# e4s2022/e4s

Hardware: AMD Instinct MI355X
Metric: 1024^2 face-swap images/sec (higher is better)
Workload: dtype f32 operands as hi+lo bf16, 3 bf16 MFMAs per product, f32 accumulate (bf16x3) on the 3x3 convs whose launch fills the chip; exact f32 elsewhere; 1 GPU; E4S-core face swap at 1024^2 (2x Net3 encoder @256^2, style swap, 12 LocalMLPs, mask-guided StyleGAN2 generator K=13), BASELINE.json configs[3] shard: 8 swaps per GPU per step; per_gpu_batch=8, global_batch=8, out_size=1024, hip_graph=True, precision=as bf16x3 where the launch fills the chip (this batch), else exact fp32, parallelism=image-parallel x1

## Files before the change

e4s_amd/csrc/conv_bf16x3.hip:

```cpp
#include "common.h"
#include <stdlib.h>

namespace {

typedef __bf16 bf16x8 __attribute__((ext_vector_type(8)));
typedef float f32x8 __attribute__((ext_vector_type(8)));

constexpr int KC = 32;
constexpr int ROWB = 144;
constexpr int LO = 64;
constexpr int TW = 16, HALO_W = TW + 2;
constexpr int PBM = 256, PTH = 16, PHALO = (PTH + 2) * HALO_W;
constexpr int PNTHR = 512;

template <int BN_, int WM_, int WN_, int TPS_, int KCH_ = 32>
struct PCfg {
    static constexpr int BN = BN_, WM = WM_, WN = WN_, TPS = TPS_, KCH = KCH_;
    static constexpr int TM = PBM / (WM * 32), TN = BN / (WN * 32);
    static constexpr int ROWB = KCH == 32 ? 144 : 80;
    static constexpr int LO = KCH * 2;
    static constexpr int QG = KCH / 8;
    static constexpr int KSTEPS = KCH / 16;
    static constexpr int ITEMS = PHALO * QG;
    static constexpr int A_BYTES = PHALO * ROWB;
// ... 43 lines not shown
    if (want > nchunk / 2) want = nchunk / 2;
    if (want < 2) return;
    cper = (nchunk + want - 1) / want;
    ksplit = (nchunk + cper - 1) / cper;
}

inline void region_split(const e4s_conv_params& p, int& ksplit, int& cper) {
    const int64_t tiles = (int64_t)p.B * ((p.Ha + 15) / 16) * ((p.Wa + 15) / 16) * p.ncls * (p.Cout / 128);
    few_tiles_split(tiles, p.Cin / 32, ksplit, cper);
}

struct TileId {
    int tb, tyb, txb, n0, ks, c_lo, c_hi;
};

template <typename C, int XF, bool SHUF, int VAR = 0>
__global__ __launch_bounds__(PNTHR) void conv_bf16x3_kernel(const e4s_conv_params p, const int ntn, const int tx_n,
                                                            const int per_img, const int ntiles, const int ksplit,
                                                            const int cper) {
    constexpr int BM = PBM, BN = C::BN, NTHR = PNTHR, WN = C::WN, TM = C::TM, TN = C::TN, TH = PTH, TPS = C::TPS;
    constexpr int NSTG = C::NSTG, PIECE = C::PIECE, BITEMS = C::BITEMS, BJ = C::BJ;
    constexpr int A_BYTES = C::A_BYTES, B_BYTES = C::B_BYTES, NZ = SHUF ? 4 : 1;
    constexpr int KC = C::KCH, ROWB = C::ROWB, LO = C::LO, QG = C::QG, KSTEPS = C::KSTEPS, BPC = C::BPC, PITEMS = C::ITEMS;
    extern __shared__ __attribute__((aligned(16))) unsigned char smem[];
    unsigned char* sA = smem;
    unsigned char* sB = smem + 2 * A_BYTES;
    int* s_out = reinterpret_cast<int*>(sB + 2 * B_BYTES);
    float* s_nz = reinterpret_cast<float*>(s_out + 3 * BM);
    double* s_st = reinterpret_cast<double*>(s_nz + 3 * BM * NZ);

    const int tid = threadIdx.x;
    const int lane = tid & 63, wave = tid >> 6;
    const int li = lane & 31, kh = lane >> 5;
    const int wm = wave / WN, wn = wave % WN;
// ... 271 lines not shown
                osc[tn] = p.out_scale ? p.out_scale[(size_t)cur.tb * p.Cout + co] : 1.f;
                bsv[tn] = p.bias ? p.bias[co] : 0.f;
                slp[tn] = (p.act == 2) ? p.slope[co] : p.alpha;
                coff[tn] = ((ph >> 1) * p.Wo + (ph & 1)) * ycs + co;
                nzi[tn] = ph;
            }
            const float gain = (p.act == 1) ? p.gain : 1.f;
            const bool do_act = p.act != 0;
            const bool raw = ksplit > 1;
            const bool stats = !SHUF && !raw && p.stats_ws != nullptr;
            double st_s[TN], st_q[TN];
#pragma unroll
            for (int tn = 0; tn < TN; ++tn) st_s[tn] = st_q[tn] = 0.0;
            float* yo = raw ? p.splitk_ws + (size_t)cur.ks * ((size_t)p.B * p.Ho * p.Wo * ycs) : p.y;
            const bool wide = (ycs & 3) == 0;
#pragma unroll
            for (int tm = 0; tm < TM; ++tm) {
#pragma unroll
                for (int g = 0; g < 4; ++g) {
                    float v[TN][4];
#pragma unroll
                    for (int i = 0; i < 4; ++i) {
                        const int r = 4 * g + i;
                        const int row = (wm * TM + tm) * 32 + i + 8 * g + 4 * kh;
                        const bool live = so[row] >= 0;
#pragma unroll
                        for (int tn = 0; tn < TN; ++tn) {
                            float t = acc[tm][tn][r];
                            if (!raw) {
                                t = t * osc[tn] + sn[row * NZ + (SHUF ? nzi[tn] : 0)] + bsv[tn];
// ... 1 lines not shown
                            }
                            v[tn][i] = t;
                            if (stats && live) { st_s[tn] += (double)t; st_q[tn] += (double)t * (double)t; }
                        }
                    }
                    if (wide) {
#pragma unroll
                        for (int tn = 0; tn < TN; ++tn) quad_transpose4(v[tn][0], v[tn][1], v[tn][2], v[tn][3], li);
                        const int off = so[(wm * TM + tm) * 32 + (li & 3) + 8 * g + 4 * kh];
                        if (off >= 0) {
#pragma unroll
                            for (int tn = 0; tn < TN; ++tn)
                                *reinterpret_cast<f32x4*>(yo + (size_t)off * ycs + coff[tn] - (li & 3)) =
                                    f32x4{v[tn][0], v[tn][1], v[tn][2], v[tn][3]};
                        }
                    } else {
#pragma unroll
                        for (int i = 0; i < 4; ++i) {
                            const int off = so[(wm * TM + tm) * 32 + i + 8 * g + 4 * kh];
                            if (off < 0) continue;
#pragma unroll
                            for (int tn = 0; tn < TN; ++tn) yo[(size_t)off * ycs + coff[tn]] = v[tn][i];
                        }
                    }
                }
            }
            if (!SHUF && stats) {
#pragma unroll
                for (int tn = 0; tn < TN; ++tn) {
                    st_s[tn] += __shfl_xor(st_s[tn], 32, 64);
                    st_q[tn] += __shfl_xor(st_q[tn], 32, 64);
                    if (kh == 0) {
                        const int col = (wn * TN + tn) * 32 + li;
                        s_st[(wm * BN + col) * 2] = st_s[tn];
                        s_st[(wm * BN + col) * 2 + 1] = st_q[tn];
                    }
                }
// ... 680 lines not shown
    few_tiles_split(tiles, p.Cin / KC, ksplit, cper);
}

int num_cus() {
    static int cus[64] = {0};
    int dev = 0;
    if (hipGetDevice(&dev) != hipSuccess) return 256;
    if (!cus[dev & 63]) {
        hipDeviceProp_t prop;
        cus[dev & 63] = (hipGetDeviceProperties(&prop, dev) == hipSuccess && prop.multiProcessorCount > 0)
                            ? prop.multiProcessorCount : 256;
    }
    return cus[dev & 63];
}

template <typename C, int XF, bool SHUF, int VAR = 0>
int launch(const e4s_conv_params& p, hipStream_t st) {
    auto kern = conv_bf16x3_kernel<C, XF, SHUF, VAR>;
    constexpr int SMEM = plain_smem<C, SHUF>();
    static_assert(SMEM <= 160 * 1024, "LDS budget");
    static std::atomic<uint64_t> smem_set{0};
    if (int e = e4s_ensure_dyn_smem(reinterpret_cast<const void*>(kern), SMEM, smem_set)) return e;
    const int ngemm = SHUF ? 4 * p.Cout : p.Cout;
    const int ntn = ngemm / C::BN;
    const int tx_n = (p.Wa + TW - 1) / TW, per_img = ((p.Ha + PTH - 1) / PTH) * tx_n;
    int ksplit, cper;
    plain_split(p, ngemm / C::BN, ksplit, cper);
    cper *= 32 / C::KCH;
    if (ksplit > 1 && !p.splitk_ws) return (int)hipErrorInvalidValue;
    const int64_t ntiles = (int64_t)p.B * per_img * ntn * ksplit;
    if (ntiles <= 0) return 0;
    if (ntiles >= (1ll << 31)) return (int)hipErrorInvalidValue;
    const int grid = (int)(ntiles < num_cus() ? ntiles : num_cus());
    hipLaunchKernelGGL(kern, dim3((unsigned)grid), dim3(PNTHR), SMEM, st, p, ntn, tx_n, per_img, (int)ntiles, ksplit, cper);
    E4S_CHECK_LAUNCH();
    if (ksplit > 1) {
        const int ycs = p.y_cstride ? p.y_cstride : p.Cout;
        const int64_t npix = (int64_t)p.B * p.Ho * p.Wo;
        const int64_t n4 = npix * (p.Cout / 4);
        hipLaunchKernelGGL(splitk_epilogue_kernel, dim3((unsigned)((n4 + 255) / 256)), dim3(256), 0, st, p, ksplit, ycs,
                           (int64_t)p.Ho * p.Wo, n4);
        E4S_CHECK_LAUNCH();
    }
    return 0;
}

template <typename C, bool SHUF>
int launch_xf(const e4s_conv_params& p, hipStream_t st) {
    if (p.in_stats) return SHUF ? (int)hipErrorInvalidValue : launch<C, 2, false>(p, st);
// ... 46 lines not shown
    }
#endif
    if (up) {
        if ((4 * p.Cout) % 128) return (int)hipErrorInvalidValue;
        return launch_xf<CfgL, true>(p, st);
    }
#ifdef E4S_ABLATIONS
    static const int k16 = [] { const char* e = getenv("E4S_PLAIN_K16"); return e ? atoi(e) : 1; }();
    if (p.Cout % 128 == 0 && !k16) return launch_xf<CfgL, false>(p, st);
#endif
    if (p.Cout % 128 == 0) return launch_xf<CfgL16, false>(p, st);
    if (p.Cout % 64 == 0) return launch_xf<CfgM, false>(p, st);
    return launch_xf<CfgS, false>(p, st);
}

int e4s_splitk_epilogue(const e4s_conv_params& p, int ksplit, hipStream_t st) {
    if (!p.splitk_ws || ksplit < 2 || p.Cout % 4) return (int)hipErrorInvalidValue;
    e4s_conv_params q = p;
    q.out_scale = nullptr;
    const int ycs = p.y_cstride ? p.y_cstride : p.Cout;
    const int64_t n4 = (int64_t)p.B * p.Ho * p.Wo * (p.Cout / 4);
    hipLaunchKernelGGL(splitk_epilogue_kernel, dim3((unsigned)((n4 + 255) / 256)), dim3(256), 0, st, q, ksplit, ycs,
                       (int64_t)p.Ho * p.Wo, n4);
    E4S_CHECK_LAUNCH();
    return 0;
}

extern "C" int64_t e4s_conv_bf16x3_ws_floats(const e4s_conv_params* pp) {
    const e4s_conv_params& p = *pp;
    if (p.istride != 1 || p.ntaps != 9 || p.Cin % KC) return 0;
// ... 24 lines not shown
```

e4s_amd/csrc/conv_c32.hip:

```cpp
#include "common.h"
#include <stdlib.h>

namespace {

typedef __bf16 bf16x8 __attribute__((ext_vector_type(8)));
typedef float f32x8 __attribute__((ext_vector_type(8)));

constexpr int KC = 32, ROWB = 128, LO = 64;
constexpr int TW = 16, TH = 16, HALO_W = TW + 2, HALO = (TH + 2) * HALO_W;
constexpr int BM = TH * TW, BN = 32, NTHR = 256;
constexpr int ITEMS = HALO * 4, AJ = (ITEMS + NTHR - 1) / NTHR;
constexpr int BPIECES = 9 * BN * 8, BJ = BPIECES / NTHR;
constexpr int A_BYTES = HALO * ROWB, B_BYTES = 9 * BN * ROWB;
constexpr int YLD = 36;
constexpr int SMEM = B_BYTES + A_BYTES + BM * 8 + 3 * BN * 4;
static_assert(BPIECES % NTHR == 0 && BM == NTHR, "thread layout");
static_assert(BM * YLD * 4 <= A_BYTES, "the output staging tile aliases the halo buffer");
static_assert(2 * SMEM <= 160 * 1024, "two blocks per CU");

__device__ __forceinline__ int swz(int r, int g) { return r * ROWB + ((g ^ ((r >> 1) & 7)) << 4); }
__device__ __forceinline__ int swz_halo(int h, int g) { return h * ROWB + ((g ^ (((h % HALO_W) >> 1) & 7)) << 4); }

__device__ __forceinline__ void split_store(unsigned char* base, int off, const f32x8 v) {
    const bf16x8 h = __builtin_convertvector(v, bf16x8);
// ... 163 lines not shown
        const float osc = p.out_scale ? p.out_scale[(size_t)cur.tb * p.Cout + co] : 1.f;
        const float bsv = p.bias ? p.bias[co] : 0.f;
        const float gain = (p.act == 1) ? p.gain : 1.f;
        const int ycs = p.y_cstride ? p.y_cstride : p.Cout;
        __syncthreads();
#pragma unroll
        for (int tm = 0; tm < 2; ++tm)
#pragma unroll
            for (int r = 0; r < 16; ++r) {
                const int row = wave * 64 + tm * 32 + (r & 3) + 8 * (r >> 2) + 4 * kh;
                float v = acc[tm][r] * osc + s_nz[row] + bsv;
                if (p.act) v = (v > 0.f ? v : v * p.alpha) * gain;
                sY[row * YLD + li] = v;
            }
        __syncthreads();
        {
            const int c4 = tid & 7;
#pragma unroll
            for (int ps = 0; ps < BM / (NTHR / 8); ++ps) {
                const int px = ps * (NTHR / 8) + (tid >> 3);
                const int off = s_out[px];
                if (off >= 0 && abl != 3)
                    *reinterpret_cast<f32x4*>(p.y + (size_t)off * ycs + cur.nt * BN + c4 * 4) =
                        *reinterpret_cast<const f32x4*>(sY + px * YLD + c4 * 4);
            }
        }
        if (RGB) {
#pragma unroll
            for (int pass = 0; pass < 2; ++pass) {
                const int px = pass * (NTHR / 2) + (tid >> 1), hf = tid & 1;
                const float* yp = sY + px * YLD + hf * 16;
// ... 126 lines not shown
    hipLaunchKernelGGL(kern, dim3((unsigned)grid), dim3(NTHR), SMEM, st, p, rgb_ws, rgb_partial, ntn, tx_n, per_img, (int)ntiles,
                       abl);
    E4S_CHECK_LAUNCH();
    return 0;
}

}

extern "C" int e4s_conv_c32_bf16x3_f32(const e4s_conv_params* pp, const float* rgb_ws, float* rgb_partial, void* stream) {
    const e4s_conv_params& p = *pp;
    if (p.Cin != KC || p.Cout % BN || p.ntaps != 9 || p.ncls != 1 || p.istride != 1 || p.ostride != 1 || p.tiles || p.labels ||
        p.in_stats || p.noise_per_channel || p.act == 2 || p.Ho != p.Hi || p.Wo != p.Wi || p.B <= 0 || p.stats_ws)
        return (int)hipErrorInvalidValue;
    if ((rgb_ws == nullptr) != (rgb_partial == nullptr) || (rgb_ws && p.Cout != BN)) return (int)hipErrorInvalidValue;
    if ((int64_t)p.B * p.Ho * p.Wo >= (1ll << 31)) return (int)hipErrorInvalidValue;
    hipStream_t st = as_stream(stream);
    if (p.in_scale) return rgb_ws ? launch<1, 1>(p, rgb_ws, rgb_partial, st) : launch<1, 0>(p, rgb_ws, rgb_partial, st);
    return rgb_ws ? launch<0, 1>(p, rgb_ws, rgb_partial, st) : launch<0, 0>(p, rgb_ws, rgb_partial, st);
}

extern "C" int e4s_torgb_finish_f32(const float* partial, const float* bias, const float* skip, const float* k4, float* out, int B,
                                    int H, int W, void* stream) {
    if (!partial || !bias || !out || (skip && (!k4 || ((H | W) & 1)))) return (int)hipErrorInvalidValue;
    if (B <= 0 || H <= 0 || W <= 0) return 0;
    const int W4 = (W + 3) / 4, HP = (H + 1) / 2;
    const int64_t n = (int64_t)B * 3 * HP * W4;
    if ((n + 255) / 256 >= (1ll << 31)) return (int)hipErrorInvalidValue;
    hipLaunchKernelGGL(torgb_finish_kernel, dim3((unsigned)((n + 255) / 256)), dim3(256), 0, as_stream(stream), partial, bias, skip, k4,
                       out, H, W, W4, HP, n);
    E4S_CHECK_LAUNCH();
    return 0;
// ... 2 lines not shown
```

e4s_amd/csrc/ops.hip:

```cpp
#include "common.h"

namespace {

__device__ __forceinline__ float bias_act_one(float x, float ref, int code, float alpha, float scale) {
    float y;
    switch (code) {
        case 12: case 32: y = 0.f; break;
        case 30: y = (x > 0.f) ? x : x * alpha; break;
        case 31: y = (ref > 0.f) ? x : x * alpha; break;
        default: y = x; break;
    }
    return y * scale;
}

__global__ void fused_bias_act_v4(const f32x4* __restrict__ x, const float* __restrict__ b,
                                  const f32x4* __restrict__ ref, f32x4* __restrict__ y, int64_t n4,
                                  int step_b, int size_b, int code, float alpha, float scale) {
    const int64_t stride = (int64_t)gridDim.x * blockDim.x;
    for (int64_t i = (int64_t)blockIdx.x * blockDim.x + threadIdx.x; i < n4; i += stride) {
        f32x4 v = x[i];
        if (b) {
            const float bv = b[((i * 4) / step_b) % size_b];
            v += bv;
        }
// ... 75 lines not shown
        if (oy >= out_h || ox >= out_w) continue;
        const int my = oy * down_y - pad_y0, mx = ox * down_x - pad_x0;
        const int iy_first = floordiv(my + up_y - 1, up_y), ix_first = floordiv(mx + up_x - 1, up_x);
        float acc = 0.f;
        for (int iy = iy_first, jy = iy_first * up_y - my; jy < kh; ++iy, jy += up_y) {
            const float* row = sx + (iy - in_y0) * tin_w;
            for (int ix = ix_first, jx = ix_first * up_x - mx; jx < kw; ++ix, jx += up_x)
                acc += row[ix - in_x0] * sk[jy * kw + jx];
        }
        y[(((int64_t)mj * out_h + oy) * out_w + ox) * minor + mi] = acc;
    }
}

}

extern "C" int e4s_abi_version(void) { return 19; }
extern "C" const char* e4s_build_arch(void) { return "gfx950"; }

extern "C" int e4s_fused_bias_act_f32(const float* x, const float* b, const float* ref, float* y, int64_t n,
                                      int step_b, int size_b, int act, int grad, float alpha, float scale,
                                      void* stream) {
    if (n <= 0) return 0;
    const int code = act * 10 + grad;
    if (code == 31 && !ref) return (int)hipErrorInvalidValue;
    if (b && (step_b <= 0 || size_b <= 0)) return (int)hipErrorInvalidValue;
    const bool vec = (n % 4 == 0) && (!b || step_b % 4 == 0) &&
                     ((reinterpret_cast<uintptr_t>(x) | reinterpret_cast<uintptr_t>(y) |
                       reinterpret_cast<uintptr_t>(ref)) % 16 == 0);
    const int block = 256;
    if (vec) {
        const int64_t n4 = n / 4;
// ... 135 lines not shown
```

e4s_amd/kernels.py:

```python
import contextlib
import ctypes
import math
import os
import threading

import torch

from . import lib
from .lib import ConvBwdParams, ConvParams, ConvWgradParams, c_p, call, fptr, ptr, stream

BM = 128
PRECISION = os.environ.get("E4S_PRECISION", "auto")
if PRECISION not in ("f32", "bf16x3", "auto"):
    raise RuntimeError(f"E4S_PRECISION must be f32, bf16x3 or auto, got {PRECISION!r}")
BF16X3_MIN_BLOCKS = int(os.environ.get("E4S_BF16X3_MIN_BLOCKS", "128"))
LRELU_GAIN = math.sqrt(2.0)


def _f32(t):
    if t.dtype != torch.float32:
        raise RuntimeError(f"expected float32 tensor, got {t.dtype}")
    return t.contiguous()


# ... 221 lines not shown


@contextlib.contextmanager
def f32_plain_split(on=True):
    prev = getattr(_split_tl, "on", False)
    _split_tl.on = bool(on)
    try:
        yield
    finally:
        _split_tl.on = prev


def conv_mfma(x, w, cout, *, plan=None, istride=1, ostride=1, ntaps=9, ncls=1, in_scale=None, out_scale=None,
              noise=None, noise_w=None, noise_per_channel=False, bias=None, slope=None, act=0, alpha=0.2,
              gain=LRELU_GAIN, spatial=None, anchors=None, labels=None, num_regions=1, w_split=None, in_stats=None,
              out=None, tap_shift=0, want_stats=False, w_split16=None, se=None):
    b, hi, wi, cin = x.shape
    if anchors is None:
        anchors = (hi // istride, wi // istride)
    ha, wa = anchors
    ho, wo = ha * ostride, wa * ostride
    if spatial is None:
        spatial = plan is None and istride == 1 and ntaps == 9
    if labels is not None and not spatial:
        raise RuntimeError("per-pixel region labels need the spatial (halo-tiled) mode")
    if plan is None and not spatial and (ha * wa) % BM != 0 and w_split is None and (in_scale is not None or out_scale is not None):
        plan = region_plan(torch.zeros(b, 1, 1, device=x.device, dtype=torch.uint8), 1, ha, wa, ncls)
    if out is None:
        y = torch.empty(b, ho, wo, cout, device=x.device, dtype=torch.float32)
    else:
        y = out
        if tuple(y.shape[:3]) != (b, ho, wo) or y.shape[3] < cout or labels is not None or plan is not None:
# ... 43 lines not shown
        if w_split16 is not None:
            if labels is None or out is not None:
                raise RuntimeError("e4s_conv_region_bf16x3_f32 is the masked-layer kernel")
            nws = lib.load().e4s_conv_region_ws_floats(ctypes.byref(p))
            if nws <= 0:
                raise RuntimeError("e4s_conv_region_bf16x3_f32 does not cover this contraction")
            skws = torch.empty(nws, device=x.device, dtype=torch.float32)
            p.splitk_ws = fptr(skws)
            global LAST_REGION_PATH
            LAST_REGION_PATH = lib.load().e4s_conv_region_path(ctypes.byref(p))
            call("e4s_conv_region_bf16x3_f32", ctypes.byref(p), ptr(w_split16), stream())
            return y
        nws = lib.load().e4s_conv_bf16x3_ws_floats(ctypes.byref(p))
        skws = torch.empty(nws, device=x.device, dtype=torch.float32) if nws else None
        p.splitk_ws = fptr(skws)
        fused = None
        if want_stats and nws == 0 and act == 0 and noise is None and out_scale is None and labels is None and ncls == 1 \
                and cout % 64 == 0 and out is None:
            if gather_ok:
                slots = (ha * wa) // 256 if (ha * wa) % 256 == 0 else 0
            else:
                slots = ((ha + 15) // 16) * ((wa + 15) // 16)
            if slots:
                fused = torch.empty(b * cout * slots * 2, device=x.device, dtype=torch.float64)
                p.stats_ws, p.stats_slots = ptr(fused), slots
        call("e4s_conv_bf16x3_f32", ctypes.byref(p), stream())
        if fused is not None:
            stats = torch.empty(b, cout, 2, device=x.device, dtype=torch.float32)
            pooled = torch.empty(b, cout, device=x.device, dtype=torch.float32)
            if se is not None:
# ... 7 lines not shown
        raise RuntimeError("fused InstanceNorm staging exists only in e4s_conv_bf16x3_f32")
    else:
        nws = lib.load().e4s_conv_mfma_ws_floats(ctypes.byref(p), 1 if spatial else 0)
        skws = torch.empty(nws, device=x.device, dtype=torch.float32) if nws else None
        p.splitk_ws = fptr(skws)
        call("e4s_conv_mfma_f32", ctypes.byref(p), 1 if spatial else 0, stream())
    if want_stats:
        stats, pooled = instnorm_stats(y, want_pooled=True)
        return y, (stats, se_gate(pooled, se[0], se[1]) if se is not None else pooled)
    return y


def bf16x3_eligible(cin, cout, *, istride=1, ostride=1, ntaps=9, ncls=1, masked=False):
    return (cin % 32 == 0 and cout % (128 if masked else 32) == 0 and istride == 1 and ntaps == 9
            and (ncls, ostride) in ((1, 1), (4, 2)))


def want_bf16x3(b, h, w, cin, cout, ncls=1, masked=False):
    if PRECISION == "f32" or not bf16x3_eligible(cin, cout, ncls=ncls, ostride=2 if ncls == 4 else 1, masked=masked):
        return False
    if PRECISION == "bf16x3":
        return True
    n = 4 * cout if (ncls == 4 and not masked) else cout
    bn = 128 if n % 128 == 0 else 64 if n % 64 == 0 else 32
    tiles = b * ((h + 15) // 16) * ((w + 15) // 16) * (n // bn) * (ncls if masked else 1)
    if tiles >= BF16X3_MIN_BLOCKS:
        return True
    nchunk = cin // 32
    split = min(nchunk // 2, -(-256 // tiles)) if nchunk >= 4 else 1
    return tiles * max(split, 1) >= 64
# ... 157 lines not shown
    p.labels, p.Hm, p.Wm = None, 0, 0
    if noise is not None:
        p.noise, p.noise_w = fptr(noise), fptr(noise_w)
        p.noise_bstride = ho * wo if noise.shape[0] > 1 else 0
    else:
        p.noise = p.noise_w = None
        p.noise_bstride = 0
    p.noise_per_channel = 0
    p.bias, p.slope = fptr(bias), None
    p.act, p.alpha, p.gain = act, alpha, gain
    call("e4s_upconv_bf16x3_f32", ctypes.byref(p), fptr(_f32(k4)), stream())
    return y


def conv_c32(x, w_split, cout, *, in_scale=None, out_scale=None, noise=None, noise_w=None, bias=None, act=0, alpha=0.2,
             gain=LRELU_GAIN, rgb_ws=None):
    b, h, w, cin = x.shape
    if cin != 32 or cout % 32:
        raise RuntimeError("conv_c32: Cin == 32 and Cout % 32 == 0")
    y = torch.empty(b, h, w, cout, device=x.device, dtype=torch.float32)
    p = ConvParams()
    p.x, p.w, p.y = fptr(x), fptr(w_split), fptr(y)
    p.y_cstride = 0
    p.rows = p.tiles = p.meta = None
    p.tiles_cap = 0
    p.B, p.Ha, p.Wa = b, h, w
    p.Hi, p.Wi, p.Ho, p.Wo, p.Cin, p.Cout = h, w, h, w, cin, cout
    p.istride, p.ostride, p.ntaps, p.ncls = 1, 1, 9, 1
    p.in_scale, p.out_scale = fptr(in_scale), fptr(out_scale)
    p.groups_per_batch = 1
    p.labels, p.Hm, p.Wm = None, 0, 0
    if noise is not None:
        p.noise, p.noise_w = fptr(noise), fptr(noise_w)
        p.noise_bstride = h * w if noise.shape[0] > 1 else 0
    else:
# ... 1035 lines not shown
```

e4s_amd/lib.py:

```python
import ctypes
import os

import torch

_HERE = os.path.dirname(os.path.abspath(__file__))
LIB_PATH = os.environ.get("E4S_LIB_PATH") or os.path.join(_HERE, "libe4s_hip.so")
ABI_VERSION = 19

c_p = ctypes.c_void_p
c_i = ctypes.c_int
c_l = ctypes.c_int64
c_f = ctypes.c_float
c_d = ctypes.c_double


STYLE_GRAD_MAX_JOBS = 32


class StyleGradJob(ctypes.Structure):
    _fields_ = [
        ("ds_raw", c_p), ("dd_d", c_p), ("d", c_p), ("s", c_p), ("wsq", c_p), ("dws", c_p), ("w3", c_p), ("wmod", c_p), ("ds_total", c_p),
        ("conv_scale", c_f), ("mod_scale", c_f), ("G", c_i), ("Cin", c_i), ("Cout", c_i), ("slot", c_i), ("masked", c_i),
    ]

# ... 61 lines not shown
    "e4s_pack_taps_f32": [c_p, c_p, c_i, c_i, c_i, c_p],
    "e4s_polyphase_weights_f32": [c_p, c_p, c_p, c_i, c_i, c_p],
    "e4s_polyphase_fold_f32": [c_p, c_p, c_p, c_i, c_i, c_p],
    "e4s_rgb_weights_f32": [c_p, c_p, c_p, c_i, c_i, c_f, c_p],
    "e4s_mask_labels": [c_p, c_p, c_p, c_i, c_i, c_i, c_i, c_p],
    "e4s_region_plan": [c_p] + [c_i] * 8 + [c_p, c_p, c_p, c_p, c_i, c_i, c_p],
    "e4s_conv_mfma_f32": [ctypes.POINTER(ConvParams), c_i, c_p],
    "e4s_upconv_mfma_f32": [ctypes.POINTER(ConvParams), c_p, c_p],
    "e4s_conv_bf16x3_f32": [ctypes.POINTER(ConvParams), c_p],
    "e4s_conv_bf16x3_ws_floats": [ctypes.POINTER(ConvParams)],
    "e4s_conv_mfma_ws_floats": [ctypes.POINTER(ConvParams), c_i],
    "e4s_split_bf16x2_f32": [c_p, c_p, c_l, c_i, c_p],
    "e4s_conv_region_bf16x3_f32": [ctypes.POINTER(ConvParams), c_p, c_p],
    "e4s_conv_region_ws_floats": [ctypes.POINTER(ConvParams)],
    "e4s_conv_region_path": [ctypes.POINTER(ConvParams)],
    "e4s_split16_bytes": [ctypes.c_int64, c_i, c_i],
    "e4s_split16_bf16x2_f32": [c_p, c_p, c_l, c_i, c_i, c_p],
    "e4s_upconv_blocks_per_cu": [],
    "e4s_instnorm_ws_doubles": [c_i, c_i, c_i],
    "e4s_conv_bwd_mfma_f32": [ctypes.POINTER(ConvBwdParams), c_p],
    "e4s_pack_taps_bwd_f32": [c_p, c_p, c_i, c_i, c_i, c_p],
    "e4s_demod_grad_f32": [c_p, c_p, c_p, c_p, c_l, c_p, c_f, c_f, c_p, c_i, c_i, c_i, c_p, c_p, c_i, c_i, c_i, c_i, c_p],
    "e4s_torgb_bwd_w_f32": [c_p, c_p, c_p, c_i, c_i, c_i, c_p, c_p, c_i, c_i, c_i, c_i, c_p],
    "e4s_conv_bwd_ws_floats": [ctypes.POINTER(ConvBwdParams)],
    "e4s_seg_reduce_nsplit": [c_i, c_i, c_i, c_i],
    "e4s_grouped_linear_t_f32": [c_p, c_p, c_p, c_p, c_i, c_i, c_i, c_i, c_f, c_p, c_p, c_p, c_f, c_p],
    "e4s_grouped_linear_t_ws_floats": [c_i, c_i, c_i, c_i],
    "e4s_reduce_parts_f32": [c_p, c_p, c_i, c_l, c_f, c_p],
    "e4s_reduce_parts_ws_floats": [c_i, c_l],
    "e4s_grouped_outer_f32": [c_p, c_p, c_p, c_i, c_i, c_i, c_i, c_f, c_p],
# ... 6 lines not shown
    "e4s_colsum_f32": [c_p, c_p, c_p, c_l, c_i, c_p],
    "e4s_colsum_ws_floats": [c_l, c_i],
    "e4s_scale_dot_f32": [c_p, c_p, c_p, c_p, c_p, c_i, c_l, c_i, c_p],
    "e4s_scale_dot_ws_floats": [c_i, c_l, c_i],
    "e4s_mask_to_u8": [c_p, c_p, c_i, c_i, c_i, c_i, c_i, c_p],
    "e4s_erode_u8": [c_p, c_p, c_i, c_i, c_i, c_i, c_i, c_p],
    "e4s_gaussian_blur_u8": [c_p, c_p, c_i, c_i, c_i, c_i, ctypes.POINTER(c_i), c_p],
    "e4s_alpha_composite_u8": [c_p, c_p, c_p, c_p, c_i, c_i, c_i, c_p],
    "e4s_pyrdown_u8": [c_p, c_p, c_i, c_i, c_i, c_i, c_p],
    "e4s_pyrdown_f32": [c_p, c_p, c_i, c_i, c_i, c_i, c_p],
    "e4s_pyrup_f32": [c_p, c_p, c_i, c_i, c_i, c_i, c_p],
    "e4s_u8_to_f32": [c_p, c_p, c_l, c_p],
    "e4s_lap_level_f32": [c_p, c_p, c_p, c_p, c_p, c_p, c_p, c_l, c_i, c_p],
    "e4s_clip_u8": [c_p, c_p, c_l, c_p],
    "e4s_conv_c32_bf16x3_f32": [c_p, c_p, c_p, c_p],
    "e4s_torgb_finish_f32": [c_p, c_p, c_p, c_p, c_p, c_i, c_i, c_i, c_p],
    "e4s_rowdot_multi_f32": [c_p, c_i, c_p, c_p, c_i, c_i, c_i, c_p],
    "e4s_ema_f32": [c_p, c_p, c_l, c_d, c_p],
    "e4s_adam_step_dev_f32": [c_p, c_p, c_p, c_p, c_l, c_d, c_p, c_d, c_d, c_d, c_d, c_p, c_p],
    "e4s_advance_i64": [c_p, c_l, c_p],
    "e4s_conv_smallcin_col2im_f32": [c_p, c_p] + [c_i] * 10 + [c_p],
    "e4s_region_scale_f32": [c_p, c_p, c_p, c_i, c_i, c_i, c_p, c_i, c_i, c_i, c_i, c_i, c_p],
    "e4s_col2im_region_nsplit": [c_i, c_i, c_i, c_i],
    "e4s_col2im_region_f32": [c_p, c_p, c_p, c_p, c_i, c_i, c_i, c_p, c_p, c_p, c_i, c_i, c_i, c_i, c_i, c_p],
    "e4s_act_bwd_demod_nsplit": [c_i, c_i, c_i, c_i],
    "e4s_act_bwd_demod_f32": [c_p, c_p, c_p, c_p, c_p, c_l, c_p, c_f, c_f, c_p, c_i, c_i, c_i, c_p, c_p, c_i, c_i, c_i, c_i, c_p],
    "e4s_pixel_unshuffle2_f32": [c_p, c_p, c_i, c_i, c_i, c_i, c_p],
    "e4s_wino_weights_bytes": [c_i, c_i],
    "e4s_wino_weights_f32": [c_p, c_p, c_i, c_i, c_p],
    "e4s_conv_wino_covers": [c_p],
# ... 145 lines not shown
```

e4s_amd/stylegan2.py:

```python
import math
import os
import random

import torch
from torch import nn
from torch.nn import functional as F

from . import kernels as K
from .op import FusedLeakyReLU, fused_leaky_relu, upfirdn2d, conv2d_gradfix


UPCONV_EXACT = os.environ.get("E4S_UPCONV", "exact") != "polyphase"
UPCONV_EXACT_MIN_RES = int(os.environ.get("E4S_UPCONV_MIN_RES", "256"))
UPCONV_BF16X3_EXACT = os.environ.get("E4S_UPCONV_BF16X3", "exact") != "polyphase"
CONV_C32 = os.environ.get("E4S_CONV_C32", "1") != "0"
REGION_ROWS = os.environ.get("E4S_REGION_ROWS", "1") != "0"


def make_kernel(k):
    k = torch.tensor(k, dtype=torch.float32)
    if k.ndim == 1:
        k = k[None, :] * k[:, None]
    return k / k.sum()


class PixelNorm(nn.Module):
    def forward(self, input):
        return input * torch.rsqrt(torch.mean(input ** 2, dim=1, keepdim=True) + 1e-8)


# ... 234 lines not shown

    def __init__(self, in_channel, out_channel, kernel_size, style_dim, upsample=False, blur_kernel=[1, 3, 3, 1],
                 demodulate=True, mask_op=False):
        super().__init__()
        self.conv = ModulatedConv2d(in_channel, out_channel, kernel_size, style_dim, upsample=upsample,
                                    blur_kernel=blur_kernel, demodulate=demodulate)
        self.noise = NoiseInjection()
        self.activate = FusedLeakyReLU(out_channel)
        self.mask_op = mask_op

    def c32_eligible(self, b, h, w, labels=None, plan=None):
        conv = self.conv
        return (CONV_C32 and not conv.upsample and labels is None and plan is None and conv.in_channel == 32
                and conv.out_channel % 32 == 0 and K.want_bf16x3(b, h, w, 32, conv.out_channel))

    def run_nhwc(self, x, s, noise, labels=None, num_regions=1, plan=None, rec=None, rgb_ws=None, d=None):
        conv = self.conv
        pk = conv.packed()
        b, h, w, _ = x.shape
        ho, wo = (2 * h, 2 * w) if conv.upsample else (h, w)
        if d is None:
            d = K.demod_coefs(s, pk["wsq"], conv.scale)
        nz, per_ch = _prep_noise(noise, b, ho, wo, x.device)
        if rec is not None:
            if per_ch:
                raise NotImplementedError("backward with per-channel noise maps")
            rec.update(d=d, noise=nz)
        ncls = 4 if conv.upsample else 1
        if not per_ch and self.c32_eligible(b, h, w, labels, plan):
            return K.conv_c32(x, conv.split_weights(), conv.out_channel, in_scale=s, out_scale=d, noise=nz,
                              noise_w=self.noise.weight, bias=self.activate.bias, act=1, alpha=self.activate.negative_slope,
                              gain=self.activate.scale, rgb_ws=rgb_ws)
        if rgb_ws is not None:
            raise RuntimeError("the fused ToRGB partial exists only on the Cin == 32 kernel")
        if (conv.upsample and labels is None and plan is None and not per_ch and UPCONV_BF16X3_EXACT
                and K.upconv_bf16x3_eligible(conv.in_channel, conv.out_channel)
                and K.want_bf16x3(b, h, w, conv.in_channel, conv.out_channel, ncls, masked=False)):
            return K.upconv_bf16x3(x, conv.subpixel_split_weights(), conv.out_channel, conv.blur.kernel, in_scale=s,
                                   out_scale=d, noise=nz, noise_w=self.noise.weight, bias=self.activate.bias, act=1,
                                   alpha=self.activate.negative_slope, gain=self.activate.scale)
        if plan is None and not per_ch and K.want_bf16x3(b, h, w, conv.in_channel, conv.out_channel, ncls,
                                                         masked=labels is not None):
            return K.conv_mfma(x, pk["w"], conv.out_channel, labels=labels, num_regions=num_regions, ncls=ncls,
                               ostride=2 if conv.upsample else 1, in_scale=s, out_scale=d, noise=nz,
                               noise_w=self.noise.weight, bias=self.activate.bias, act=1,
                               alpha=self.activate.negative_slope, gain=self.activate.scale,
                               w_split=conv.split_weights(),
                               w_split16=conv.split_weights16() if (labels is not None and REGION_ROWS) else None)
        if conv.upsample and plan is None and UPCONV_EXACT and (labels is None or ho >= UPCONV_EXACT_MIN_RES):
# ... 256 lines not shown
        if soft and tape is not None:
            raise NotImplementedError("backward with soft (non one-hot) masks")

        sp = None
        if not soft and lat.shape[3] == 512:
            sp = self._style_plan(b, r, lat.shape[2], lat.device)
            sbuf = torch.empty(sp["s_floats"], device=lat.device, dtype=torch.float32)
            dbuf = torch.empty(sp["d_floats"], device=lat.device, dtype=torch.float32)
            K.rowdot_multi(*sp["s"], lat, sbuf, 0)
            K.rowdot_multi(*sp["d"], sbuf, dbuf, 1)

        def pre(layer, which):
            off, g, c = sp["meta"][id(layer)][which]
            return (sbuf if which == "s" else dbuf)[off:off + g * c].view(g, c)

        def styled(layer, x, idx, nz, rgb_ws=None):
            mod = layer.conv.modulation
            s = pre(layer, "s") if sp is not None else K.modulate(lat, idx, layer.mask_op, mod.weight, mod.bias)
            if soft and layer.mask_op:
                return layer.run_nhwc_soft(x, s, nz, mask)
            rec = {} if tape is not None else None
            y = layer.run_nhwc(x, s, nz, labels if layer.mask_op else None, r, rec=rec, rgb_ws=rgb_ws,
                               d=pre(layer, "d") if sp is not None else None)
            partial = None
            if rgb_ws is not None:
                y, partial = y
            if tape is not None:
                rec.update(kind="conv", layer=layer, idx=idx, masked=layer.mask_op, x=x, y=y, s=s,
                           labels=labels if layer.mask_op else None)
                tape.append(rec)
            return y if rgb_ws is None else (y, partial)

        def styled_then_rgb(conv2, to_rgb, x, idx, nz, skip):
            mod = to_rgb.conv.modulation
            s_rgb = pre(to_rgb, "s") if sp is not None else K.modulate(lat, idx + 1, False, mod.weight, mod.bias)
            ws = K.rgb_weights(to_rgb.conv.packed()["w"].view(3, -1), s_rgb, to_rgb.conv.scale)
            y, partial = styled(conv2, x, idx, nz, rgb_ws=ws)
            out = K.torgb_finish(partial, to_rgb.bias, skip, to_rgb.upsample.kernel if skip is not None else None)
            if tape is not None:
                tape.append(dict(kind="rgb", layer=to_rgb, idx=idx + 1, masked=False, x=y, s=s_rgb, ws=ws,
                                 has_skip=skip is not None, out=out, labels=None))
            return y, out

        def rgb(layer, x, idx, skip):
            mod = layer.conv.modulation
            s = pre(layer, "s") if sp is not None else K.modulate(lat, idx, layer.mask_op, mod.weight, mod.bias)
            if soft and layer.mask_op:
                return layer.run_nhwc_soft(x, s, mask, skip)
            rec = {} if tape is not None else None
            out = layer.run_nhwc(x, s, labels if layer.mask_op else None, r, skip, rec=rec)
            if tape is not None:
                rec.update(kind="rgb", layer=layer, idx=idx, masked=layer.mask_op, x=x, s=s, has_skip=skip is not None, out=out,
                           labels=labels if layer.mask_op else None)
                tape.append(rec)
            return out

        x = K.const_input(self.input.input, b)
        x = styled(self.conv1, x, 0, noise[0])
        skip = rgb(self.to_rgb1, x, 1, None)
        feats = None
        i = 1
        for conv1, conv2, to_rgb in zip(self.convs[::2], self.convs[1::2], self.to_rgbs):
            x = styled(conv1, x, i, noise[i])
            if i + 2 == self.split_layer_idx:
                feats = K.nhwc_to_nchw(x)
                if tape is not None:
                    tape[-1]["is_feats"] = True
            nz2 = noise[i + 1]
            if (not soft and not conv2.mask_op and not to_rgb.mask_op and conv2.conv.out_channel == 32
                    and (nz2 is None or nz2.shape[1] == 1) and conv2.c32_eligible(b, x.shape[1], x.shape[2])):
                x, skip = styled_then_rgb(conv2, to_rgb, x, i + 1, nz2, skip)
            else:
                x = styled(conv2, x, i + 1, nz2)
                skip = rgb(to_rgb, x, i + 2, skip)
            i += 2
        return skip, feats


def _packed_equal_conv(conv, cin_pad):
    key = _param_key(conv.weight) + (cin_pad,)
    pk = getattr(conv, "_e4s_pack", None)
    if pk is None or pk["key"] != key:
        with torch.no_grad():
            w = conv.weight.detach().float() * conv.scale
            cout, cin, k, _ = w.shape
# ... 144 lines not shown
```

include/e4s_hip.h:

```cpp
#ifndef E4S_HIP_H
#define E4S_HIP_H
#include <stdint.h>

#ifdef __cplusplus
extern "C" {
#endif

int e4s_abi_version(void);
const char* e4s_build_arch(void);


int e4s_fused_bias_act_f32(const float* x, const float* b, const float* ref, float* y, int64_t n,
                           int step_b, int size_b, int act, int grad, float alpha, float scale,
                           void* stream);

int e4s_upfirdn2d_f32(const float* x, const float* k, float* y, int major, int in_h, int in_w, int minor,
                      int kh, int kw, int up_x, int up_y, int down_x, int down_y,
                      int pad_x0, int pad_x1, int pad_y0, int pad_y1, void* stream);

int e4s_channel_sum_f32(const float* g, float* out, int64_t n, int step_b, int size_b, void* stream);


int e4s_rowdot_f32(const float* in, int64_t in_stride, const float* M, const float* bias, float* out,
                   int G, int O, int K, int mode, float scale, void* stream);
// ... 55 lines not shown
    float* splitk_ws;
    double* stats_ws;
    int stats_slots;
    int tap_shift;
    int split_hint;
} e4s_conv_params;

int e4s_conv_mfma_f32(const e4s_conv_params* p, int spatial, void* stream);
int64_t e4s_conv_mfma_ws_floats(const e4s_conv_params* p, int spatial);

int e4s_upconv_mfma_f32(const e4s_conv_params* p, const float* k4, void* stream);
int e4s_upconv_blocks_per_cu(void);

int e4s_conv_bf16x3_f32(const e4s_conv_params* p, void* stream);
int64_t e4s_conv_bf16x3_ws_floats(const e4s_conv_params* p);
int e4s_split_bf16x2_f32(const float* w, void* out, int64_t rows, int cin, void* stream);

int e4s_conv_region_bf16x3_f32(const e4s_conv_params* p, const void* w16, void* stream);
int64_t e4s_conv_region_ws_floats(const e4s_conv_params* p);
int e4s_conv_region_path(const e4s_conv_params* p);
int e4s_split16_bf16x2_f32(const float* w, void* out, int64_t rows, int cout, int cin, void* stream);
int64_t e4s_split16_bytes(int64_t rows, int cout, int cin);

typedef struct {
    const float* gz;
    const float* wt;
    float* dx;
    const float* x;
    float* ds;
    const float* s;
// ... 284 lines not shown
```

Before: 487.7 images/s.

## Fuse ToRGB into Cout=64 bf16x3 conv epilogue and skip final activation store

Adds an RGB variant of the plain bf16x3 conv kernel whose epilogue stages each 64-channel output tile in a spare LDS A buffer and computes the modulated 1x1 ToRGB partial in-kernel. This lets the 512^2 Cout=64 layer feed torgb_finish directly instead of running a separate ToRGB conv that rereads the activation. Separately, the last Cin=32 conv can now skip writing its activation when no tape is recorded, since only the RGB output is consumed. The fused path adds wave barriers, a block sync and extra registers to the epilogue, and it only applies when no split-K is used.

```diff
diff --git a/e4s_amd/csrc/conv_bf16x3.hip b/e4s_amd/csrc/conv_bf16x3.hip
--- a/e4s_amd/csrc/conv_bf16x3.hip
+++ b/e4s_amd/csrc/conv_bf16x3.hip
@@ -81,10 +81,11 @@
     int tb, tyb, txb, n0, ks, c_lo, c_hi;
 };
 
-template <typename C, int XF, bool SHUF, int VAR = 0>
+template <typename C, int XF, bool SHUF, int VAR = 0, bool RGB = false>
 __global__ __launch_bounds__(PNTHR) void conv_bf16x3_kernel(const e4s_conv_params p, const int ntn, const int tx_n,
                                                             const int per_img, const int ntiles, const int ksplit,
-                                                            const int cper) {
+                                                            const int cper, const float* __restrict__ rgb_ws,
+                                                            float* __restrict__ rgb_partial) {
     constexpr int BM = PBM, BN = C::BN, NTHR = PNTHR, WN = C::WN, TM = C::TM, TN = C::TN, TH = PTH, TPS = C::TPS;
     constexpr int NSTG = C::NSTG, PIECE = C::PIECE, BITEMS = C::BITEMS, BJ = C::BJ;
     constexpr int A_BYTES = C::A_BYTES, B_BYTES = C::B_BYTES, NZ = SHUF ? 4 : 1;
@@ -386,6 +387,21 @@
             for (int tn = 0; tn < TN; ++tn) st_s[tn] = st_q[tn] = 0.0;
             float* yo = raw ? p.splitk_ws + (size_t)cur.ks * ((size_t)p.B * p.Ho * p.Wo * ycs) : p.y;
             const bool wide = (ycs & 3) == 0;
+            constexpr int RLD = 36;
+            static_assert(!RGB || (TN == 1 && WN == 2 && BN == 64 && !SHUF && (PNTHR / 64) * 32 * RLD * 4 <= A_BYTES &&
+                                   BM * 3 * 4 <= C::WM * BN * 2 * 8), "ToRGB epilogue: 64-column tile, staging inside one A buffer");
+            float* sR = reinterpret_cast<float*>(sA + ((cg + 1) & 1) * A_BYTES) + wave * 32 * RLD;
+            float* sP = reinterpret_cast<float*>(s_st);
+            const int rrow = lane >> 1, rhf = lane & 1;
+            f32x4 rw[3][4];
+            float ra[TM][3];
+            if (RGB) {
+                const float* wsb = rgb_ws + (size_t)cur.tb * 3 * BN + wn * 32 + rhf * 16;
+#pragma unroll
+                for (int c = 0; c < 3; ++c)
+#pragma unroll
+                    for (int q = 0; q < 4; ++q) rw[c][q] = *reinterpret_cast<const f32x4*>(wsb + c * BN + q * 4);
+            }
 #pragma unroll
             for (int tm = 0; tm < TM; ++tm) {
 #pragma unroll
@@ -417,6 +433,9 @@
                                 *reinterpret_cast<f32x4*>(yo + (size_t)off * ycs + coff[tn] - (li & 3)) =
                                     f32x4{v[tn][0], v[tn][1], v[tn][2], v[tn][3]};
                         }
+                        if (RGB)
+                            *reinterpret_cast<f32x4*>(sR + ((li & 3) + 8 * g + 4 * kh) * RLD + (li & ~3)) =
+                                f32x4{v[0][0], v[0][1], v[0][2], v[0][3]};
                     } else {
 #pragma unroll
                         for (int i = 0; i < 4; ++i) {
@@ -424,6 +443,48 @@
                             if (off < 0) continue;
 #pragma unroll
                             for (int tn = 0; tn < TN; ++tn) yo[(size_t)off * ycs + coff[tn]] = v[tn][i];
+                        }
+                    }
+                }
+                if (RGB) {
+                    __builtin_amdgcn_fence(__ATOMIC_RELEASE, "wavefront");
+                    __builtin_amdgcn_wave_barrier();
+                    __builtin_amdgcn_fence(__ATOMIC_ACQUIRE, "wavefront");
+                    const float* yp = sR + rrow * RLD + rhf * 16;
+                    float a0 = 0.f, a1 = 0.f, a2 = 0.f;
+#pragma unroll
+                    for (int q = 0; q < 4; ++q) {
+                        const f32x4 t = *reinterpret_cast<const f32x4*>(yp + q * 4);
+                        a0 += t[0] * rw[0][q][0] + t[1] * rw[0][q][1] + t[2] * rw[0][q][2] + t[3] * rw[0][q][3];
+                        a1 += t[0] * rw[1][q][0] + t[1] * rw[1][q][1] + t[2] * rw[1][q][2] + t[3] * rw[1][q][3];
+                        a2 += t[0] * rw[2][q][0] + t[1] * rw[2][q][1] + t[2] * rw[2][q][2] + t[3] * rw[2][q][3];
+                    }
+                    ra[tm][0] = a0 + __shfl_xor(a0, 1, 64);
+                    ra[tm][1] = a1 + __shfl_xor(a1, 1, 64);
+                    ra[tm][2] = a2 + __shfl_xor(a2, 1, 64);
+                    __builtin_amdgcn_fence(__ATOMIC_RELEASE, "wavefront");
+                    __builtin_amdgcn_wave_barrier();
+                }
+            }
+            if (RGB) {
+                if (wn == 1 && rhf == 0) {
+#pragma unroll
+                    for (int tm = 0; tm < TM; ++tm)
+#pragma unroll
+                        for (int c = 0; c < 3; ++c) sP[((wm * TM + tm) * 32 + rrow) * 3 + c] = ra[tm][c];
+                }
+                __syncthreads();
+                if (wn == 0 && rhf == 0) {
+                    const int HWo = p.Ho * p.Wo;
+#pragma unroll
+                    for (int tm = 0; tm < TM; ++tm) {
+                        const int prow = (wm * TM + tm) * 32 + rrow;
+                        const int off = so[prow];
+                        if (off >= 0) {
+                            float* o = rgb_partial + (size_t)cur.tb * 3 * HWo + (off - cur.tb * HWo);
+                            o[0] = ra[tm][0] + sP[prow * 3];
+                            o[HWo] = ra[tm][1] + sP[prow * 3 + 1];
+                            o[2 * (size_t)HWo] = ra[tm][2] + sP[prow * 3 + 2];
                         }
                     }
                 }
@@ -1134,9 +1195,9 @@
     return cus[dev & 63];
 }
 
-template <typename C, int XF, bool SHUF, int VAR = 0>
-int launch(const e4s_conv_params& p, hipStream_t st) {
-    auto kern = conv_bf16x3_kernel<C, XF, SHUF, VAR>;
+template <typename C, int XF, bool SHUF, int VAR = 0, bool RGB = false>
+int launch(const e4s_conv_params& p, hipStream_t st, const float* rgb_ws = nullptr, float* rgb_partial = nullptr) {
+    auto kern = conv_bf16x3_kernel<C, XF, SHUF, VAR, RGB>;
     constexpr int SMEM = plain_smem<C, SHUF>();
     static_assert(SMEM <= 160 * 1024, "LDS budget");
     static std::atomic<uint64_t> smem_set{0};
@@ -1148,11 +1209,13 @@
     plain_split(p, ngemm / C::BN, ksplit, cper);
     cper *= 32 / C::KCH;
     if (ksplit > 1 && !p.splitk_ws) return (int)hipErrorInvalidValue;
+    if (RGB && (ksplit > 1 || ntn != 1 || !rgb_ws || !rgb_partial)) return (int)hipErrorInvalidValue;
     const int64_t ntiles = (int64_t)p.B * per_img * ntn * ksplit;
     if (ntiles <= 0) return 0;
     if (ntiles >= (1ll << 31)) return (int)hipErrorInvalidValue;
     const int grid = (int)(ntiles < num_cus() ? ntiles : num_cus());
-    hipLaunchKernelGGL(kern, dim3((unsigned)grid), dim3(PNTHR), SMEM, st, p, ntn, tx_n, per_img, (int)ntiles, ksplit, cper);
+    hipLaunchKernelGGL(kern, dim3((unsigned)grid), dim3(PNTHR), SMEM, st, p, ntn, tx_n, per_img, (int)ntiles, ksplit, cper,
+                       rgb_ws, rgb_partial);
     E4S_CHECK_LAUNCH();
     if (ksplit > 1) {
         const int ycs = p.y_cstride ? p.y_cstride : p.Cout;
@@ -1229,6 +1292,27 @@
     return launch_xf<CfgS, false>(p, st);
 }
 
+static bool rgb_covers(const e4s_conv_params& p) {
+    if (p.Cin % KC || p.Cout != 64 || p.ntaps != 9 || p.ncls != 1 || p.istride != 1 || p.ostride != 1 || p.tiles || p.labels ||
+        p.noise_per_channel || p.in_stats || p.stats_ws || p.act == 2 || p.Ha != p.Hi || p.Wa != p.Wi || p.Ho != p.Hi || p.Wo != p.Wi ||
+        p.B <= 0 || (p.y_cstride & 3) || (p.y_cstride && p.y_cstride < p.Cout) || !p.x || !p.w || !p.y)
+        return false;
+    if ((int64_t)p.B * p.Ho * p.Wo >= (1ll << 31)) return false;
+    int ksplit, cper;
+    plain_split(p, 1, ksplit, cper);
+    return ksplit == 1;
+}
+
+extern "C" int e4s_conv_bf16x3_rgb_ok(const e4s_conv_params* pp) { return rgb_covers(*pp) ? 1 : 0; }
+
+extern "C" int e4s_conv_bf16x3_rgb_f32(const e4s_conv_params* pp, const float* rgb_ws, float* rgb_partial, void* stream) {
+    const e4s_conv_params& p = *pp;
+    if (!rgb_ws || !rgb_partial || !rgb_covers(p)) return (int)hipErrorInvalidValue;
+    hipStream_t st = as_stream(stream);
+    return p.in_scale ? launch<CfgM, 1, false, 0, true>(p, st, rgb_ws, rgb_partial)
+                      : launch<CfgM, 0, false, 0, true>(p, st, rgb_ws, rgb_partial);
+}
+
 int e4s_splitk_epilogue(const e4s_conv_params& p, int ksplit, hipStream_t st) {
     if (!p.splitk_ws || ksplit < 2 || p.Cout % 4) return (int)hipErrorInvalidValue;
     e4s_conv_params q = p;
diff --git a/e4s_amd/csrc/conv_c32.hip b/e4s_amd/csrc/conv_c32.hip
--- a/e4s_amd/csrc/conv_c32.hip
+++ b/e4s_amd/csrc/conv_c32.hip
@@ -201,7 +201,7 @@
                 sY[row * YLD + li] = v;
             }
         __syncthreads();
-        {
+        if (RGB != 2) {
             const int c4 = tid & 7;
 #pragma unroll
             for (int ps = 0; ps < BM / (NTHR / 8); ++ps) {
@@ -358,7 +358,9 @@
         return (int)hipErrorInvalidValue;
     if ((rgb_ws == nullptr) != (rgb_partial == nullptr) || (rgb_ws && p.Cout != BN)) return (int)hipErrorInvalidValue;
     if ((int64_t)p.B * p.Ho * p.Wo >= (1ll << 31)) return (int)hipErrorInvalidValue;
+    if (!p.x || !p.w || (!p.y && !rgb_ws)) return (int)hipErrorInvalidValue;
     hipStream_t st = as_stream(stream);
+    if (rgb_ws && !p.y) return p.in_scale ? launch<1, 2>(p, rgb_ws, rgb_partial, st) : launch<0, 2>(p, rgb_ws, rgb_partial, st);
     if (p.in_scale) return rgb_ws ? launch<1, 1>(p, rgb_ws, rgb_partial, st) : launch<1, 0>(p, rgb_ws, rgb_partial, st);
     return rgb_ws ? launch<0, 1>(p, rgb_ws, rgb_partial, st) : launch<0, 0>(p, rgb_ws, rgb_partial, st);
 }
diff --git a/e4s_amd/csrc/ops.hip b/e4s_amd/csrc/ops.hip
--- a/e4s_amd/csrc/ops.hip
+++ b/e4s_amd/csrc/ops.hip
@@ -113,7 +113,7 @@
 
 }
 
-extern "C" int e4s_abi_version(void) { return 19; }
+extern "C" int e4s_abi_version(void) { return 20; }
 extern "C" const char* e4s_build_arch(void) { return "gfx950"; }
 
 extern "C" int e4s_fused_bias_act_f32(const float* x, const float* b, const float* ref, float* y, int64_t n,
diff --git a/e4s_amd/kernels.py b/e4s_amd/kernels.py
--- a/e4s_amd/kernels.py
+++ b/e4s_amd/kernels.py
@@ -259,8 +259,10 @@
 def conv_mfma(x, w, cout, *, plan=None, istride=1, ostride=1, ntaps=9, ncls=1, in_scale=None, out_scale=None,
               noise=None, noise_w=None, noise_per_channel=False, bias=None, slope=None, act=0, alpha=0.2,
               gain=LRELU_GAIN, spatial=None, anchors=None, labels=None, num_regions=1, w_split=None, in_stats=None,
-              out=None, tap_shift=0, want_stats=False, w_split16=None, se=None):
+              out=None, tap_shift=0, want_stats=False, w_split16=None, se=None, rgb_ws=None):
     b, hi, wi, cin = x.shape
+    if rgb_ws is not None and (w_split is None or w_split16 is not None or want_stats or tuple(rgb_ws.shape) != (b, 3, cout)):
+        raise RuntimeError("conv_mfma(rgb_ws=...): the fused ToRGB partial exists on the plain split-bf16 kernel, rgb_ws [B,3,Cout]")
     if anchors is None:
         anchors = (hi // istride, wi // istride)
     ha, wa = anchors
@@ -334,6 +336,12 @@
         nws = lib.load().e4s_conv_bf16x3_ws_floats(ctypes.byref(p))
         skws = torch.empty(nws, device=x.device, dtype=torch.float32) if nws else None
         p.splitk_ws = fptr(skws)
+        if rgb_ws is not None:
+            if not lib.load().e4s_conv_bf16x3_rgb_ok(ctypes.byref(p)):
+                raise RuntimeError("e4s_conv_bf16x3_rgb_f32 does not cover this contraction")
+            partial = torch.empty(b, 3, ho, wo, device=x.device, dtype=torch.float32)
+            call("e4s_conv_bf16x3_rgb_f32", ctypes.byref(p), fptr(rgb_ws), fptr(partial), stream())
+            return y, partial
         fused = None
         if want_stats and nws == 0 and act == 0 and noise is None and out_scale is None and labels is None and ncls == 1 \
                 and cout % 64 == 0 and out is None:
@@ -371,6 +379,11 @@
 def bf16x3_eligible(cin, cout, *, istride=1, ostride=1, ntaps=9, ncls=1, masked=False):
     return (cin % 32 == 0 and cout % (128 if masked else 32) == 0 and istride == 1 and ntaps == 9
             and (ncls, ostride) in ((1, 1), (4, 2)))
+
+
+def bf16x3_rgb_eligible(b, h, w, cin, cout):
+    tiles = b * ((h + 15) // 16) * ((w + 15) // 16)
+    return cout == 64 and cin % 32 == 0 and (cin // 32 < 4 or tiles > 128)
 
 
 def want_bf16x3(b, h, w, cin, cout, ncls=1, masked=False):
@@ -558,11 +571,13 @@
 
 
 def conv_c32(x, w_split, cout, *, in_scale=None, out_scale=None, noise=None, noise_w=None, bias=None, act=0, alpha=0.2,
-             gain=LRELU_GAIN, rgb_ws=None):
+             gain=LRELU_GAIN, rgb_ws=None, store_y=True):
     b, h, w, cin = x.shape
     if cin != 32 or cout % 32:
         raise RuntimeError("conv_c32: Cin == 32 and Cout % 32 == 0")
-    y = torch.empty(b, h, w, cout, device=x.device, dtype=torch.float32)
+    if not store_y and rgb_ws is None:
+        raise RuntimeError("conv_c32: store_y=False leaves nothing to return without rgb_ws")
+    y = torch.empty(b, h, w, cout, device=x.device, dtype=torch.float32) if store_y else None
     p = ConvParams()
     p.x, p.w, p.y = fptr(x), fptr(w_split), fptr(y)
     p.y_cstride = 0
diff --git a/e4s_amd/lib.py b/e4s_amd/lib.py
--- a/e4s_amd/lib.py
+++ b/e4s_amd/lib.py
@@ -5,7 +5,7 @@
 
 _HERE = os.path.dirname(os.path.abspath(__file__))
 LIB_PATH = os.environ.get("E4S_LIB_PATH") or os.path.join(_HERE, "libe4s_hip.so")
-ABI_VERSION = 19
+ABI_VERSION = 20
 
 c_p = ctypes.c_void_p
 c_i = ctypes.c_int
@@ -99,6 +99,7 @@
     "e4s_conv_region_bf16x3_f32": [ctypes.POINTER(ConvParams), c_p, c_p],
     "e4s_conv_region_ws_floats": [ctypes.POINTER(ConvParams)],
     "e4s_conv_region_path": [ctypes.POINTER(ConvParams)],
+    "e4s_conv_bf16x3_rgb_ok": [ctypes.POINTER(ConvParams)],
     "e4s_split16_bytes": [ctypes.c_int64, c_i, c_i],
     "e4s_split16_bf16x2_f32": [c_p, c_p, c_l, c_i, c_i, c_p],
     "e4s_upconv_blocks_per_cu": [],
@@ -135,6 +136,7 @@
     "e4s_lap_level_f32": [c_p, c_p, c_p, c_p, c_p, c_p, c_p, c_l, c_i, c_p],
     "e4s_clip_u8": [c_p, c_p, c_l, c_p],
     "e4s_conv_c32_bf16x3_f32": [c_p, c_p, c_p, c_p],
+    "e4s_conv_bf16x3_rgb_f32": [c_p, c_p, c_p, c_p],
     "e4s_torgb_finish_f32": [c_p, c_p, c_p, c_p, c_p, c_i, c_i, c_i, c_p],
     "e4s_rowdot_multi_f32": [c_p, c_i, c_p, c_p, c_i, c_i, c_i, c_p],
     "e4s_ema_f32": [c_p, c_p, c_l, c_d, c_p],
diff --git a/e4s_amd/stylegan2.py b/e4s_amd/stylegan2.py
--- a/e4s_amd/stylegan2.py
+++ b/e4s_amd/stylegan2.py
@@ -14,6 +14,8 @@
 UPCONV_EXACT_MIN_RES = int(os.environ.get("E4S_UPCONV_MIN_RES", "256"))
 UPCONV_BF16X3_EXACT = os.environ.get("E4S_UPCONV_BF16X3", "exact") != "polyphase"
 CONV_C32 = os.environ.get("E4S_CONV_C32", "1") != "0"
+C32_SKIP_Y = os.environ.get("E4S_C32_SKIP_Y", "1") != "0"
+TORGB_FUSED64 = os.environ.get("E4S_TORGB_FUSED64", "1") != "0"
 REGION_ROWS = os.environ.get("E4S_REGION_ROWS", "1") != "0"
 
 
@@ -278,7 +280,13 @@
         return (CONV_C32 and not conv.upsample and labels is None and plan is None and conv.in_channel == 32
                 and conv.out_channel % 32 == 0 and K.want_bf16x3(b, h, w, 32, conv.out_channel))
 
-    def run_nhwc(self, x, s, noise, labels=None, num_regions=1, plan=None, rec=None, rgb_ws=None, d=None):
+    def rgb64_eligible(self, b, h, w, labels=None, plan=None):
+        conv = self.conv
+        return (TORGB_FUSED64 and not conv.upsample and labels is None and plan is None and conv.out_channel == 64
+                and not (CONV_C32 and conv.in_channel == 32)
+                and K.want_bf16x3(b, h, w, conv.in_channel, 64) and K.bf16x3_rgb_eligible(b, h, w, conv.in_channel, 64))
+
+    def run_nhwc(self, x, s, noise, labels=None, num_regions=1, plan=None, rec=None, rgb_ws=None, d=None, store_y=True):
         conv = self.conv
         pk = conv.packed()
         b, h, w, _ = x.shape
@@ -294,9 +302,15 @@
         if not per_ch and self.c32_eligible(b, h, w, labels, plan):
             return K.conv_c32(x, conv.split_weights(), conv.out_channel, in_scale=s, out_scale=d, noise=nz,
                               noise_w=self.noise.weight, bias=self.activate.bias, act=1, alpha=self.activate.negative_slope,
-                              gain=self.activate.scale, rgb_ws=rgb_ws)
+                              gain=self.activate.scale, rgb_ws=rgb_ws, store_y=store_y)
+        if not store_y:
+            raise RuntimeError("only the Cin == 32 kernel runs without storing its activation")
         if rgb_ws is not None:
-            raise RuntimeError("the fused ToRGB partial exists only on the Cin == 32 kernel")
+            if per_ch or not self.rgb64_eligible(b, h, w, labels, plan):
+                raise RuntimeError("the fused ToRGB partial exists only on the Cin == 32 kernel and the Cout == 64 plain kernel")
+            return K.conv_mfma(x, pk["w"], conv.out_channel, in_scale=s, out_scale=d, noise=nz, noise_w=self.noise.weight,
+                               bias=self.activate.bias, act=1, alpha=self.activate.negative_slope, gain=self.activate.scale,
+                               w_split=conv.split_weights(), rgb_ws=rgb_ws)
         if (conv.upsample and labels is None and plan is None and not per_ch and UPCONV_BF16X3_EXACT
                 and K.upconv_bf16x3_eligible(conv.in_channel, conv.out_channel)
                 and K.want_bf16x3(b, h, w, conv.in_channel, conv.out_channel, ncls, masked=False)):
@@ -583,14 +597,14 @@
             off, g, c = sp["meta"][id(layer)][which]
             return (sbuf if which == "s" else dbuf)[off:off + g * c].view(g, c)
 
-        def styled(layer, x, idx, nz, rgb_ws=None):
+        def styled(layer, x, idx, nz, rgb_ws=None, store_y=True):
             mod = layer.conv.modulation
             s = pre(layer, "s") if sp is not None else K.modulate(lat, idx, layer.mask_op, mod.weight, mod.bias)
             if soft and layer.mask_op:
                 return layer.run_nhwc_soft(x, s, nz, mask)
             rec = {} if tape is not None else None
             y = layer.run_nhwc(x, s, nz, labels if layer.mask_op else None, r, rec=rec, rgb_ws=rgb_ws,
-                               d=pre(layer, "d") if sp is not None else None)
+                               d=pre(layer, "d") if sp is not None else None, store_y=store_y)
             partial = None
             if rgb_ws is not None:
                 y, partial = y
@@ -600,11 +614,11 @@
                 tape.append(rec)
             return y if rgb_ws is None else (y, partial)
 
-        def styled_then_rgb(conv2, to_rgb, x, idx, nz, skip):
+        def styled_then_rgb(conv2, to_rgb, x, idx, nz, skip, store_y=True):
             mod = to_rgb.conv.modulation
             s_rgb = pre(to_rgb, "s") if sp is not None else K.modulate(lat, idx + 1, False, mod.weight, mod.bias)
             ws = K.rgb_weights(to_rgb.conv.packed()["w"].view(3, -1), s_rgb, to_rgb.conv.scale)
-            y, partial = styled(conv2, x, idx, nz, rgb_ws=ws)
+            y, partial = styled(conv2, x, idx, nz, rgb_ws=ws, store_y=store_y)
             out = K.torgb_finish(partial, to_rgb.bias, skip, to_rgb.upsample.kernel if skip is not None else None)
             if tape is not None:
                 tape.append(dict(kind="rgb", layer=to_rgb, idx=idx + 1, masked=False, x=y, s=s_rgb, ws=ws,
@@ -629,15 +643,19 @@
         skip = rgb(self.to_rgb1, x, 1, None)
         feats = None
         i = 1
-        for conv1, conv2, to_rgb in zip(self.convs[::2], self.convs[1::2], self.to_rgbs):
+        npairs = len(self.to_rgbs)
+        for pair, (conv1, conv2, to_rgb) in enumerate(zip(self.convs[::2], self.convs[1::2], self.to_rgbs)):
             x = styled(conv1, x, i, noise[i])
             if i + 2 == self.split_layer_idx:
                 feats = K.nhwc_to_nchw(x)
                 if tape is not None:
                     tape[-1]["is_feats"] = True
             nz2 = noise[i + 1]
-            if (not soft and not conv2.mask_op and not to_rgb.mask_op and conv2.conv.out_channel == 32
-                    and (nz2 is None or nz2.shape[1] == 1) and conv2.c32_eligible(b, x.shape[1], x.shape[2])):
+            fusable = not soft and not conv2.mask_op and not to_rgb.mask_op and (nz2 is None or nz2.shape[1] == 1)
+            if fusable and conv2.conv.out_channel == 32 and conv2.c32_eligible(b, x.shape[1], x.shape[2]):
+                x, skip = styled_then_rgb(conv2, to_rgb, x, i + 1, nz2, skip,
+                                          store_y=not (C32_SKIP_Y and tape is None and pair == npairs - 1))
+            elif fusable and conv2.rgb64_eligible(b, x.shape[1], x.shape[2]):
                 x, skip = styled_then_rgb(conv2, to_rgb, x, i + 1, nz2, skip)
             else:
                 x = styled(conv2, x, i + 1, nz2)
diff --git a/include/e4s_hip.h b/include/e4s_hip.h
--- a/include/e4s_hip.h
+++ b/include/e4s_hip.h
@@ -93,6 +93,8 @@
 
 int e4s_conv_bf16x3_f32(const e4s_conv_params* p, void* stream);
 int64_t e4s_conv_bf16x3_ws_floats(const e4s_conv_params* p);
+int e4s_conv_bf16x3_rgb_f32(const e4s_conv_params* p, const float* rgb_ws, float* rgb_partial, void* stream);
+int e4s_conv_bf16x3_rgb_ok(const e4s_conv_params* p);
 int e4s_split_bf16x2_f32(const float* w, void* out, int64_t rows, int cin, void* stream);
 
 int e4s_conv_region_bf16x3_f32(const e4s_conv_params* p, const void* w16, void* stream);
```

Measured after the change: 490.3 images/s, median of 3. Within noise of the previous version (+0.5%).
